# armadaproject/armada

Measured on AMD Instinct MI355X. Metric: scheduling rounds/sec (p99 round latency in p99_ms), 100k nodes x 1M jobs, higher is better.
Workload: dtype int64; 1 GPU; BASELINE configs[2]: 100000 nodes x 64 queues x 1000000 queued jobs (+560757 running), R=4, 3 priority classes, DRF weights, global burst 200000, queue burst 20000, protectedFractionOfFairShare 0.5; nodes=100000, queued_jobs=1000000, running_jobs=560757, queues=64, parallelism=1 pool on 1 gpu, seed=20260921

## Files before the change

### armada_amd/csrc/engine_hc.h

```cpp
#pragma once

#define HC_CMDS 32
#define HC_INS 16
enum { HC_Q = 1, HC_I, HC_D, HC_C, HC_E };
struct alignas(16) HcCmd { int32_t type, a; uint64_t fieldMin; int64_t ex0, ex1; int32_t cls, seq; uint64_t pad[2]; };
struct alignas(16) HcRep { int32_t seq, slot; uint64_t key; int32_t node, insDone; int64_t ex0, ex1; uint64_t cls; uint64_t pad; };
struct alignas(16) HcIns { uint64_t key; int32_t node, pad; int64_t ex0, ex1; uint64_t cls; uint64_t pad2[2]; };
struct HcBox {
  int32_t cmdPub, cmdDone, overflow, insDone;
  unsigned long long clb[128];
  int32_t scratch[64];
  int16_t freeStack[512];
  int32_t insSlot[HC_CMDS];
  HcCmd cmd[HC_CMDS]; HcRep rep[4]; HcIns ins[HC_INS];
};
static_assert(sizeof(HcCmd) == 64 && sizeof(HcRep) == 64 && sizeof(HcIns) == 64, "HC mailbox records are 64 bytes");
static_assert(sizeof(HcBox) <= sizeof(g_fl.evWin), "the HC mailbox lives in the idle key windows");
#define HCB (*(HcBox*)&g_fl.evWin[0][0])
#define HC_ROWS (L0CAP / 64)
#define HC_H_MAX 48

__device__ static inline unsigned hcMin32(unsigned v) {
  asm volatile(
      "s_nop 1\n\tv_min_u32_dpp %0, %0, %0 row_shr:1 row_mask:0xf bank_mask:0xf\n\t"
      "s_nop 1\n\tv_min_u32_dpp %0, %0, %0 row_shr:2 row_mask:0xf bank_mask:0xf\n\t"
      "s_nop 1\n\tv_min_u32_dpp %0, %0, %0 row_shr:4 row_mask:0xf bank_mask:0xf\n\t"
      "s_nop 1\n\tv_min_u32_dpp %0, %0, %0 row_shr:8 row_mask:0xf bank_mask:0xf\n\t"
      "s_nop 1\n\tv_min_u32_dpp %0, %0, %0 row_bcast:15 row_mask:0xa bank_mask:0xf\n\t"
      "s_nop 1\n\tv_min_u32_dpp %0, %0, %0 row_bcast:31 row_mask:0xc bank_mask:0xf\n\t"
      "s_nop 1"
      : "+v"(v));
  return (unsigned)__builtin_amdgcn_readlane((int)v, 63);
}
__device__ static inline unsigned long long hcMinKey(unsigned long long key, int* laneOut) {
  const unsigned hi = (unsigned)(key >> 32), lo = (unsigned)key;
  const unsigned mh = hcMin32(hi);
  const unsigned ml = hcMin32(hi == mh ? lo : 0xffffffffu);
  const unsigned long long mn = ((unsigned long long)mh << 32) | ml;
  const unsigned long long who = __ballot(key == mn);
  *laneOut = mn == ~0ull ? -1 : (int)__builtin_ctzll(who | (1ull << 63));
  return mn;
}
__device__ static inline unsigned long long hcRead64(unsigned long long v, int lane) { return slGet64(v, lane); }
__device__ static inline int hcLoadI32(const int32_t* p) { return __builtin_amdgcn_readfirstlane(__hip_atomic_load(p, __ATOMIC_RELAXED, __HIP_MEMORY_SCOPE_WORKGROUP)); }
__device__ static inline void hcStoreI32(int32_t* p, int v) { __hip_atomic_store(p, v, __ATOMIC_RELAXED, __HIP_MEMORY_SCOPE_WORKGROUP); }
struct HcNeed { unsigned long long fmin; long long ex0, ex1; int cls; };
template <int E> __device__ static inline bool hcFits(unsigned long long G, const HcNeed& q, unsigned long long key, unsigned long long cls, long long ex0, long long ex1) {
  bool ok = ((cls >> q.cls) & 1) != 0;
  ok &= (((key | G) - q.fmin) & G) == G;
  if (E > 0) ok &= q.ex0 <= ex0;
  if (E > 1) ok &= q.ex1 <= ex1;
  return ok;
}

struct HcRows { unsigned long long key[HC_ROWS], cls[HC_ROWS]; long long ex0[HC_ROWS], ex1[HC_ROWS]; };
template <int R> __device__ static inline void hcRowSet(HcRows& rows, int lane, unsigned long long key, long long ex0, long long ex1, unsigned long long cls) {
  if ((int)(threadIdx.x & 63) == lane) { rows.key[R] = key; rows.ex0[R] = ex0; rows.ex1[R] = ex1; rows.cls[R] = cls; }
}
__device__ static inline void hcRowSetAt(HcRows& rows, int slot, unsigned long long key, long long ex0, long long ex1, unsigned long long cls) {
  const int lane = slot & 63;
  switch (slot >> 6) {
#define HC_CASE(R) case R: hcRowSet<R>(rows, lane, key, ex0, ex1, cls); break;
    HC_CASE(0) HC_CASE(1) HC_CASE(2) HC_CASE(3) HC_CASE(4) HC_CASE(5) HC_CASE(6) HC_CASE(7) HC_CASE(8) HC_CASE(9) HC_CASE(10) HC_CASE(11) HC_CASE(12) HC_CASE(13) HC_CASE(14) HC_CASE(15)
#undef HC_CASE
  }
}
static_assert(HC_ROWS == 16, "hcRowSetAt enumerates the rows");

template <int E> __device__ static void coldSession(Dev& d, KREF k) {
  (void)d;
  const int lane = threadIdx.x & 63;
  const unsigned long long G = UNI64(k.guardMask);
  HcRows rows;
  int hi = __builtin_amdgcn_readfirstlane(g_fl.l0Count);
  int nfree = 0, insDone = 0, overflow = 0;
  ShapeReq sq[2];
#pragma unroll
  for (int x = 0; x < 2; x++) { const int t = lane + 64 * x; if (t < k.S) sq[x] = d.shapeTab[t]; else { sq[x].fieldMin = 0; sq[x].ex0 = sq[x].ex1 = 0; sq[x].cls = 0; sq[x].never = 1; } }
#pragma unroll
  for (int r = 0; r < HC_ROWS; r++) {
    const int s = r * 64 + lane;
    const bool in = s < hi;
    rows.key[r] = in ? g_fl.l0Key[s] : ~0ull; rows.ex0[r] = in ? g_fl.l0Ex0[s] : 0; rows.ex1[r] = in ? g_fl.l0Ex1[s] : 0; rows.cls[r] = in ? g_fl.l0Cls[s] : 0ull;
  }
  int done = 0;
  unsigned spins = 0;
  const int debugHang = d.f.debugHang;
#ifdef ASCHED_FASTPROF
  long long cBusy = 0, cT0 = 0; int cQ = 0, cI = 0;
#endif
  for (;;) {
    const HcCmd& c = HCB.cmd[done & (HC_CMDS - 1)];
    const int pubV = __hip_atomic_load(&HCB.cmdPub, __ATOMIC_RELAXED, __HIP_MEMORY_SCOPE_WORKGROUP);
    LDS_ORDER();
    const int typeV = c.type, aV = c.a, seqV = c.seq;
    HcNeed q; q.fmin = c.fieldMin; q.ex0 = c.ex0; q.ex1 = c.ex1; q.cls = c.cls;
    if (__builtin_amdgcn_readfirstlane(pubV) == done) { __builtin_amdgcn_s_sleep(1); if (waitGaveUp(spins)) return; continue; }
    spins = 0;
    if (debugHang > 0 && done == debugHang) { for (;;) { __builtin_amdgcn_s_sleep(1); if (waitGaveUp(spins)) return; } }
#ifdef ASCHED_FASTPROF
    cT0 = CLK();
#endif
    {
      const int type = __builtin_amdgcn_readfirstlane(typeV), a = __builtin_amdgcn_readfirstlane(aV);
      if (type == HC_Q) {
#ifdef ASCHED_FASTPROF
        cQ++;
#endif
        const int seq = __builtin_amdgcn_readfirstlane(seqV);
        unsigned long long best = ~0ull; int bs = -1;
        const int nrows = (hi + 63) >> 6;
#pragma unroll
        for (int rr = 0; rr < HC_ROWS; rr++) {
          if (rr < nrows) {
            const bool ok = hcFits<E>(G, q, rows.key[rr], rows.cls[rr], rows.ex0[rr], rows.ex1[rr]) & (rows.key[rr] < best);
            best = ok ? rows.key[rr] : best; bs = ok ? rr * 64 + lane : bs;
          }
        }
        int bl;
        const unsigned long long mn = hcMinKey(best, &bl);
        const int slot = bl >= 0 ? __builtin_amdgcn_readlane(bs, bl) : -1;
        HcRep& o = HCB.rep[seq & 3];
        if (lane == 0) { o.slot = slot; o.key = mn; o.insDone = overflow ? -1 : insDone; HCB.clb[a & 127] = mn; }
        LDS_ORDER();
        hcStoreI32(&o.seq, seq);
      } else if (type == HC_I) {
#ifdef ASCHED_FASTPROF
        cI++;
#endif
        const HcIns& in = HCB.ins[a & (HC_INS - 1)];
        const unsigned long long key = UNI64(in.key), cls = UNI64(in.cls); const long long ex0 = (long long)UNI64(in.ex0), ex1 = (long long)UNI64(in.ex1);
        const int node = __builtin_amdgcn_readfirstlane(in.node);
        int slot;
        if (nfree > 0) { nfree--; slot = __builtin_amdgcn_readfirstlane((int)HCB.freeStack[nfree]); }
        else if (hi < L0CAP) slot = hi++;
        else slot = -1;
        if (slot < 0) overflow = 1;
        else {
          if (lane == 0) { g_fl.l0Key[slot] = key; g_fl.l0Node[slot] = node; g_fl.l0Ex0[slot] = ex0; g_fl.l0Ex1[slot] = ex1; g_fl.l0Cls[slot] = cls; g_fl.l0Cls2[slot] = 0; HCB.insSlot[a & (HC_CMDS - 1)] = slot; }
          LANE0_PUBLISHED();
          hcRowSetAt(rows, slot, key, ex0, ex1, cls);
#pragma unroll
          for (int x = 0; x < 2; x++) {
            HcNeed nq; nq.fmin = sq[x].fieldMin; nq.ex0 = sq[x].ex0; nq.ex1 = sq[x].ex1; nq.cls = sq[x].cls;
            if (!sq[x].never && hcFits<E>(G, nq, key, cls, ex0, ex1)) (void)__hip_atomic_fetch_min(&HCB.clb[lane + 64 * x], key, __ATOMIC_RELAXED, __HIP_MEMORY_SCOPE_WORKGROUP);
          }
        }
        insDone = a + 1;
        LDS_ORDER();
        hcStoreI32(&HCB.insDone, overflow ? -1 : insDone);
      } else if (type == HC_D || type == HC_C) {
        const int slot = type == HC_D ? a : __builtin_amdgcn_readfirstlane(HCB.insSlot[a & (HC_CMDS - 1)]);
        if (slot >= 0) {
          if (lane == 0) { const int nd = g_fl.l0Node[slot]; if (nd >= 0) k.l0Slot[nd] = -1; g_fl.l0Node[slot] = -1; if (nfree < 512) HCB.freeStack[nfree] = (int16_t)slot; }
          LANE0_PUBLISHED();
          if (nfree < 512) nfree++;
          hcRowSetAt(rows, slot, ~0ull, 0, 0, 0ull);
        }
      } else if (type == HC_E) {
        int base = 0;
        const int nrows = (hi + 63) >> 6;
#pragma unroll
        for (int rr = 0; rr < HC_ROWS; rr++) {
          if (rr < nrows) {
            const int s = rr * 64 + lane;
            const int node = s < hi ? g_fl.l0Node[s] : -1;
            const bool valid = node >= 0;
            const unsigned long long b = __ballot(valid);
            const int dst = base + __popcll(b & ((1ull << lane) - 1));
            LDS_ORDER();
            if (valid) { g_fl.l0Key[dst] = rows.key[rr]; g_fl.l0Node[dst] = node; g_fl.l0Ex0[dst] = rows.ex0[rr]; g_fl.l0Ex1[dst] = rows.ex1[rr]; g_fl.l0Cls[dst] = rows.cls[rr]; g_fl.l0Cls2[dst] = 0; k.l0Slot[node] = dst; }
            LDS_ORDER();
            base += __popcll(b);
          }
        }
        if (lane == 0) g_fl.l0Count = base;
        LANE0_PUBLISHED();
#ifdef ASCHED_FASTPROF
        cBusy += CLK() - cT0;
        if (lane == 0) { g_rs.statSeg[24] += cBusy; g_rs.statSeg[25] += cQ * 1000ll; g_rs.statSeg[26] += cI * 1000ll; g_rs.statSeg[27] += (long long)hi * 1000; g_rs.statSeg[28] += 1000; }
#endif
        __builtin_amdgcn_fence(__ATOMIC_RELEASE, "agent");
        LDS_ORDER();
        hcStoreI32(&HCB.cmdDone, done + 1);
        return;
      }
      LDS_ORDER();
      done++;
    }
#ifdef ASCHED_FASTPROF
    cBusy += CLK() - cT0;
#endif
  }
}
__device__ static void coldLoop(Dev& d) {
  const FastK k = fastKRef(d);
  int gen = 0;
  unsigned spins = 0;
  for (;;) {
    for (;;) {
      int g = hcLoadI32(&g_fl.eng.hcGen);
      if (g != gen) { gen = g; break; }
      if (hcLoadI32(&g_fl.eng.bindQuit)) return;
      __builtin_amdgcn_s_sleep(2);
      if (waitGaveUp(spins)) return;
    }
    spins = 0;
    LDS_ORDER();
    if (k.E == 0) coldSession<0>(d, k); else if (k.E == 1) coldSession<1>(d, k); else coldSession<2>(d, k);
  }
}

struct HcHot { unsigned long long key, cls; long long ex0, ex1; int node, state, seq; };
enum { SC_NONE = 0, SC_SCAN = 1, SC_HEAD = 2 };
struct HcShapes { int pos[2], st[2], node[2], wIdx[2]; unsigned long long w[2], key[2], cls[2], lb[2]; long long ex0[2], ex1[2];
                  int pos2[2], node2[2]; unsigned long long key2[2], cls2[2]; long long ex02[2], ex12[2]; unsigned long long bk[2]; };
__device__ static inline void hcShapesBound(HcShapes& sc, unsigned long long on) {
#pragma unroll
  for (int x = 0; x < 2; x++) {
    const unsigned long long b = sc.st[x] == SC_HEAD ? sc.key[x] : (sc.st[x] == SC_SCAN ? sc.lb[x] : ~0ull);
    sc.bk[x] = b & on;
  }
}
__device__ static inline void hcShapesLoad(KREF k, HcShapes& sc) {
  const int lane = threadIdx.x & 63;
#pragma unroll
  for (int x = 0; x < 2; x++) {
    const int s = lane + 64 * x;
    sc.st[x] = SC_NONE; sc.pos[x] = 0; sc.node[x] = -1; sc.wIdx[x] = -1; sc.w[x] = 0; sc.key[x] = 0; sc.cls[x] = 0; sc.lb[x] = 0; sc.ex0[x] = 0; sc.ex1[x] = 0;
    sc.pos2[x] = -1; sc.node2[x] = -1; sc.key2[x] = 0; sc.cls2[x] = 0; sc.ex02[x] = 0; sc.ex12[x] = 0;
    if (s < k.S) {
      const CandRec c = g_fl.cand[s];
      if (c.node >= 0) { sc.st[x] = SC_HEAD; sc.pos[x] = c.pos; sc.node[x] = c.node; sc.key[x] = c.key; sc.cls[x] = c.cls; sc.ex0[x] = c.ex0; sc.ex1[x] = c.ex1; }
      else if (c.node == -2) { sc.st[x] = SC_SCAN; sc.pos[x] = c.pos + (c.key != 0 ? 1 : 0); sc.lb[x] = c.key; }
    }
  }
}
__device__ static inline void hcShapesStore(KREF k, const HcShapes& sc) {
  const int lane = threadIdx.x & 63;
#pragma unroll
  for (int x = 0; x < 2; x++) {
    const int s = lane + 64 * x;
    if (s < k.S) {
      CandRec c; c.pad = 0;
      if (sc.st[x] == SC_HEAD) { c.pos = sc.pos[x]; c.node = sc.node[x]; c.key = sc.key[x]; c.cls = sc.cls[x]; c.ex0 = sc.ex0[x]; c.ex1 = sc.ex1[x]; }
      else if (sc.st[x] == SC_SCAN) { c.node = -2; c.key = sc.lb[x]; c.pos = sc.lb[x] != 0 ? sc.pos[x] - 1 : sc.pos[x]; c.cls = 0; c.ex0 = c.ex1 = 0; }
      else { c.node = -1; c.pos = k.N; c.key = 0; c.cls = 0; c.ex0 = c.ex1 = 0; }
      g_fl.cand[s] = c;
    }
  }
}
__device__ static inline void hcShapesUsed(HcShapes& sc, int P) {
  const int wi = P >> 6; const unsigned long long bit = 1ull << (P & 63);
#pragma unroll
  for (int x = 0; x < 2; x++) {
    sc.w[x] = sc.wIdx[x] == wi ? sc.w[x] & ~bit : sc.w[x];
    const bool was = (sc.st[x] == SC_HEAD) & (sc.pos[x] == P);
    const bool promote = was & (sc.pos2[x] >= 0);
    const bool scan = was & !promote;
    sc.lb[x] = was ? sc.key[x] : sc.lb[x];
    sc.key[x] = promote ? sc.key2[x] : sc.key[x]; sc.cls[x] = promote ? sc.cls2[x] : sc.cls[x]; sc.node[x] = promote ? sc.node2[x] : sc.node[x];
    sc.ex0[x] = promote ? sc.ex02[x] : sc.ex0[x]; sc.ex1[x] = promote ? sc.ex12[x] : sc.ex1[x];
    sc.pos[x] = promote ? sc.pos2[x] : (scan ? P + 1 : sc.pos[x]); sc.st[x] = scan ? SC_SCAN : sc.st[x];
    sc.pos2[x] = (promote | (sc.pos2[x] == P)) ? -1 : sc.pos2[x];
  }
}
__device__ static inline void hcShapesFetch(KREF k, FastS& ES, HcShapes& sc, int target) {
  const int lane = threadIdx.x & 63;
  const int tx = target >> 6, tl = target & 63;
  for (;;) {
    unsigned long long nw[2]; bool needW[2];
#pragma unroll
    for (int x = 0; x < 2; x++) {
      const int s = lane + 64 * x, wi = sc.pos[x] >> 6;
      if (sc.st[x] == SC_SCAN && wi >= k.fitW) sc.st[x] = SC_NONE;
      needW[x] = sc.st[x] == SC_SCAN && sc.wIdx[x] != wi;
      nw[x] = 0;
      if (needW[x]) nw[x] = __hip_atomic_load(&k.fitBits[(size_t)s * k.fitW + wi], __ATOMIC_RELAXED, __HIP_MEMORY_SCOPE_AGENT);
    }
    ES.statScanSteps++;
    unsigned long long fKey[2], fCls[2]; long long fEx0[2], fEx1[2]; int fNode[2], fRem[2], hp[2]; bool needF[2];
    unsigned long long gKey[2], gCls[2]; long long gEx0[2], gEx1[2]; int gNode[2], gRem[2], hp2[2]; bool needG[2];
#pragma unroll
    for (int x = 0; x < 2; x++) {
      const int wi = sc.pos[x] >> 6;
      if (needW[x]) { sc.w[x] = nw[x]; sc.wIdx[x] = wi; }
      const unsigned long long m = sc.st[x] == SC_SCAN ? sc.w[x] & (~0ull << (sc.pos[x] & 63)) : 0ull;
      needF[x] = m != 0;
      hp[x] = wi * 64 + (int)__builtin_ctzll(m | (1ull << 63));
      if (sc.st[x] == SC_SCAN && m == 0) sc.pos[x] = (wi + 1) << 6;
      fKey[x] = 0; fCls[x] = 0; fEx0[x] = 0; fEx1[x] = 0; fNode[x] = -1; fRem[x] = 1;
      if (needF[x]) {
        const int q = hp[x];
        fRem[x] = (int)__hip_atomic_load(&k.baseRemoved[q], __ATOMIC_RELAXED, __HIP_MEMORY_SCOPE_AGENT);
        fKey[x] = k.baseKey[q]; fCls[x] = k.baseCls[q]; fNode[x] = k.baseNode[q];
        fEx0[x] = k.E > 0 ? k.baseExtra[q] : 0; fEx1[x] = k.E > 1 ? k.baseExtra[k.Npad + q] : 0;
      }
      const unsigned long long m2 = m & (m - 1);
      needG[x] = needF[x] & (m2 != 0);
      hp2[x] = wi * 64 + (int)__builtin_ctzll(m2 | (1ull << 63));
      gKey[x] = 0; gCls[x] = 0; gEx0[x] = 0; gEx1[x] = 0; gNode[x] = -1; gRem[x] = 1;
      if (needG[x]) {
        const int q = hp2[x];
        gRem[x] = (int)__hip_atomic_load(&k.baseRemoved[q], __ATOMIC_RELAXED, __HIP_MEMORY_SCOPE_AGENT);
        gKey[x] = k.baseKey[q]; gCls[x] = k.baseCls[q]; gNode[x] = k.baseNode[q];
        gEx0[x] = k.E > 0 ? k.baseExtra[q] : 0; gEx1[x] = k.E > 1 ? k.baseExtra[k.Npad + q] : 0;
      }
    }
#pragma unroll
    for (int x = 0; x < 2; x++) {
      if (needF[x]) {
        if (fRem[x]) { sc.w[x] &= ~(1ull << (hp[x] & 63)); sc.pos[x] = hp[x] + 1; }
        else {
          sc.st[x] = SC_HEAD; sc.pos[x] = hp[x]; sc.key[x] = fKey[x]; sc.cls[x] = fCls[x]; sc.node[x] = fNode[x]; sc.ex0[x] = fEx0[x]; sc.ex1[x] = fEx1[x];
          const bool sp = needG[x] & (gRem[x] == 0);
          sc.pos2[x] = sp ? hp2[x] : -1; sc.key2[x] = gKey[x]; sc.cls2[x] = gCls[x]; sc.node2[x] = gNode[x]; sc.ex02[x] = gEx0[x]; sc.ex12[x] = gEx1[x];
        }
      }
    }
    const int ts = tx ? __builtin_amdgcn_readlane(sc.st[1], tl) : __builtin_amdgcn_readlane(sc.st[0], tl);
    if (ts != SC_SCAN) return;
  }
}

struct HcJobV { unsigned long long keyDelta, fmin; long long ex0, ex1; int cls, never, rq, pub, shape; };
__device__ static inline void hcLoadEntry(int idx, HcJobV& o) {
  o.pub = __hip_atomic_load(&g_fl.eng.ringPub, __ATOMIC_RELAXED, __HIP_MEMORY_SCOPE_WORKGROUP);
  LDS_ORDER();
  o.rq = RQ(idx);
  const JobTail& t = *(const JobTail*)&RREC(idx).keyDelta;
  o.keyDelta = t.keyDelta; o.fmin = t.fieldMin; o.cls = t.cls; o.never = (int)t.never; o.ex0 = t.ex0; o.ex1 = t.ex1; o.shape = t.shape;
}
__device__ static inline void hcPostQ(int& cmdPub, const HcJobV& j, int seq) {
  HcCmd& c = HCB.cmd[cmdPub & (HC_CMDS - 1)];
  if ((threadIdx.x & 63) == 0) { c.type = HC_Q; c.a = j.shape; c.seq = seq; c.fieldMin = j.fmin; c.ex0 = j.ex0; c.ex1 = j.ex1; c.cls = j.cls; }
  LDS_ORDER();
  cmdPub++;
  hcStoreI32(&HCB.cmdPub, cmdPub);
}
__device__ static inline void hcPostA(int& cmdPub, int type, int a) {
  HcCmd& c = HCB.cmd[cmdPub & (HC_CMDS - 1)];
  if ((threadIdx.x & 63) == 0) { c.type = type; c.a = a; }
  LDS_ORDER();
  cmdPub++;
  hcStoreI32(&HCB.cmdPub, cmdPub);
}

__device__ static inline int hcHotBind(HcHot& h, int hLane, const HcJobV& j, unsigned long long G, unsigned long long MFM, long long ME0, long long ME1) {
  const unsigned long long nk = h.key - j.keyDelta; const long long n0 = h.ex0 - j.ex0, n1 = h.ex1 - j.ex1;
  const bool alive = ((((nk | G) - MFM) & G) == G) & (ME0 <= n0) & (ME1 <= n1);
  const bool me = (int)(threadIdx.x & 63) == hLane;
  h.key = me ? (alive ? nk : ~0ull) : h.key; h.ex0 = me ? n0 : h.ex0; h.ex1 = me ? n1 : h.ex1; h.state = me ? (alive ? 1 : 0) : h.state; h.cls = (me & !alive) ? 0ull : h.cls;
  return __ballot(me & !alive) ? 1 : 0;
}
#define HC_ERR_SHORT 610

struct HcOut { int engSeq, statScanSteps, statL0Max, hcShort; long long segT, eseg[8]; };
template <int E> __device__ static __attribute__((noinline)) HcOut engineStreamHcT(Dev& d, const FastK k, const int engSeq0, const int statScan0, const int statL0Max0, const long long segT0) {
  FastS ES; ES.engSeq = engSeq0; ES.statScanSteps = statScan0; ES.statL0Max = statL0Max0; ES.segT = segT0; ES.laneL = 0; ES.laneX = 0;
#ifdef ASCHED_FASTPROF
  for (int x = 0; x < 8; x++) ES.eseg[x] = 0;
#endif
  const int lane = threadIdx.x & 63;
  const unsigned long long G = UNI64(k.guardMask), MFM = UNI64(k.minFieldMin);
  const long long ME0 = (long long)UNI64(k.minEx0), ME1 = (long long)UNI64(k.minEx1);
  if (lane == 0) { HCB.cmdPub = 0; HCB.cmdDone = 0; HCB.overflow = 0; HCB.insDone = 0; for (int x = 0; x < 4; x++) HCB.rep[x].seq = -1; }
  HCB.clb[lane] = 0; HCB.clb[lane + 64] = 0;
  LDS_ORDER();
  hcStoreI32(&g_fl.eng.hcGen, __builtin_amdgcn_readfirstlane(g_fl.eng.hcGen) + 1);
  int cmdPub = 0, insSeq = 0, rrNext = 0, qSeq = 0, inFlight = 0;
  HcHot h; h.key = ~0ull; h.cls = 0; h.ex0 = h.ex1 = 0; h.node = -1; h.state = 0; h.seq = 0;
  const unsigned long long shortOn = d.f.hcShort ? ~0ull : 0ull;
  HcShapes sc; hcShapesLoad(k, sc); hcShapesBound(sc, shortOn);
  int nShort = 0;
  int total = __builtin_amdgcn_readfirstlane(g_fl.l0Count);
  int i = 0, fail = 0;
  HcJobV cur; bool haveCur = false;
#ifdef ASCHED_FASTPROF
  int pSrc[4] = {0, 0, 0, 0}, pFetch = 0, pDry = 0, pAsk = 0;
#endif
#ifdef ASCHED_HC_CHECK
  int chkNode = -1, chkQ = 0, chkScan = 0;
#endif
  for (;;) {
    if (!haveCur) {
#ifdef ASCHED_FASTPROF
      pDry++;
#endif
      for (;;) {
        hcLoadEntry(i, cur);
        if (__builtin_amdgcn_readfirstlane(cur.pub) > i) break;
        if (hcLoadI32(&g_fl.eng.ringEnd) | hcLoadI32(&g_fl.eng.abandon)) { hcLoadEntry(i, cur); break; }
        __builtin_amdgcn_s_sleep(1);
      }
      if (__builtin_amdgcn_readfirstlane(cur.pub) <= i) break;
      haveCur = true;
    }
    ESEG(0);
    const int flags = __builtin_amdgcn_readfirstlane((cur.rq & RQ_EV) | (cur.never << 16));
    if (flags) {
      if (flags >> 16) { fail = 1; break; }
      i++; haveCur = false;
      hcStoreI32(&g_fl.eng.ringAck, i);
      continue;
    }
    if ((++ES.engSeq & 255) == 0 && cancelRequested(d)) { if (lane == 0) g_fl.eng.cancel = 1; LANE0_PUBLISHED(); fail = 1; break; }
    HcJobV nxt; hcLoadEntry(i + 1, nxt);
    const int rIns = __hip_atomic_load(&HCB.insDone, __ATOMIC_RELAXED, __HIP_MEMORY_SCOPE_WORKGROUP);
    LDS_ORDER();
    const unsigned long long rLb = HCB.clb[cur.shape & 127];
    HcNeed q; q.fmin = cur.fmin; q.ex0 = cur.ex0; q.ex1 = cur.ex1; q.cls = cur.cls;
    const bool fitH = hcFits<E>(G, q, h.key, h.cls, h.ex0, h.ex1);
    int hLane;
    unsigned long long hk = hcMinKey(fitH ? h.key : ~0ull, &hLane);
    const int shape = __builtin_amdgcn_readfirstlane(cur.shape), sl = shape & 63;
    const bool hiSet = cur.shape >= 64;
    ESEG(1);
    int insDone = __builtin_amdgcn_readfirstlane(rIns);
    if (insDone < 0) { fail = 2; break; }
    if (inFlight > 0) {
      const bool rel = (h.state == 2) & (h.seq < insDone);
      const unsigned long long rb = __ballot(rel);
      h.state = rel ? 0 : h.state; h.cls = rel ? 0ull : h.cls; h.key = rel ? ~0ull : h.key;
      inFlight -= __popcll(rb);
      const bool drop = hLane >= 0 && ((rb >> hLane) & 1);
      hLane = drop ? -1 : hLane; hk = drop ? ~0ull : hk;
    }
    {
      const unsigned long long bkS = hcRead64(hiSet ? sc.bk[1] : sc.bk[0], sl);
      const int stH = __builtin_amdgcn_readlane(h.state, hLane & 63);
#ifdef ASCHED_HC_CHECK
      chkNode = -1; chkQ = qSeq; chkScan = ES.statScanSteps;
      if (!(rLb < hk) & (hk < bkS) & (stH == 1)) chkNode = __builtin_amdgcn_readlane(h.node, hLane & 63);
#else
      if (!(rLb < hk) & (hk < bkS) & (stH == 1)) {
        RREC(i).node0 = __builtin_amdgcn_readlane(h.node, hLane & 63);
        LDS_ORDER();
        i++;
        hcStoreI32(&g_fl.eng.ringAck, i);
        total -= hcHotBind(h, hLane, cur, G, MFM, ME0, ME1);
        nShort++;
        cur = nxt; haveCur = __builtin_amdgcn_readfirstlane(nxt.pub) > i;
        ESEG(6);
        continue;
      }
#endif
    }
    int cst = __builtin_amdgcn_readlane(hiSet ? sc.st[1] : sc.st[0], sl);
    unsigned long long cKey = hcRead64(hiSet ? sc.key[1] : sc.key[0], sl);
    const unsigned long long cLb = hcRead64(hiSet ? sc.lb[1] : sc.lb[0], sl);
    const unsigned long long ckLb = UNI64(rLb);
    const unsigned long long known = cst == SC_HEAD && cKey < hk ? cKey : hk;
    unsigned long long ck = ~0ull; int cSlot = -1;
    if (ckLb < known) {
#ifdef ASCHED_FASTPROF
      pAsk++;
#endif
      hcPostQ(cmdPub, cur, qSeq);
      HcRep& rp = HCB.rep[qSeq & 3];
      for (;;) { if ((int)(hcLoadI32(&rp.seq) == qSeq) | hcLoadI32(&g_fl.eng.abandon)) break; __builtin_amdgcn_s_sleep(1); }
      LDS_ORDER();
      qSeq++;
      cSlot = __builtin_amdgcn_readfirstlane(rp.slot); ck = UNI64(rp.key);
      insDone = __builtin_amdgcn_readfirstlane(rp.insDone) | -hcLoadI32(&g_fl.eng.abandon);
      if (insDone < 0) { fail = 2; break; }
      const bool rel = (h.state == 2) & (h.seq < insDone);
      const unsigned long long rb = __ballot(rel);
      h.state = rel ? 0 : h.state; h.cls = rel ? 0ull : h.cls; h.key = rel ? ~0ull : h.key;
      inFlight -= __popcll(rb);
      const bool drop = hLane >= 0 && ((rb >> hLane) & 1);
      hLane = drop ? -1 : hLane; hk = drop ? ~0ull : hk;
    }
    ESEG(2);
    const unsigned long long lk = hk < ck ? hk : ck;
    if (cst == SC_SCAN && !(lk < cLb)) {
#ifdef ASCHED_FASTPROF
      pFetch++;
#endif
      hcShapesFetch(k, ES, sc, shape);
      hcShapesBound(sc, shortOn);
      cst = __builtin_amdgcn_readlane(hiSet ? sc.st[1] : sc.st[0], sl);
      cKey = hcRead64(hiSet ? sc.key[1] : sc.key[0], sl);
    }
    const unsigned long long lk2 = hk < ck ? hk : ck;
    const unsigned long long bk = cst == SC_HEAD ? cKey : (cst == SC_SCAN ? cLb : ~0ull);
    const bool dirtyWins = lk2 < bk;
    if (!dirtyWins & (cst != SC_HEAD)) { fail = 1; break; }
    const int src = dirtyWins ? (hk < ck ? 0 : 1) : 2;
    const int nH = __builtin_amdgcn_readlane(h.node, hLane & 63), nB = __builtin_amdgcn_readlane(hiSet ? sc.node[1] : sc.node[0], sl);
    int n = dirtyWins ? nH : nB;
    if (src == 1) n = __builtin_amdgcn_readfirstlane(g_fl.l0Node[cSlot]);
#ifdef ASCHED_HC_CHECK
    if (chkNode >= 0) {
      if ((src != 0) | (n != chkNode) | (qSeq != chkQ) | (ES.statScanSteps != chkScan)) { if (lane == 0 && RS.error == 0) { RS.error = ASCHED_ERR_INTERNAL; RS.errorDetail = HC_ERR_SHORT; } LANE0_PUBLISHED(); fail = 1; break; }
      nShort++;
    }
#endif
#ifdef ASCHED_FASTPROF
    pSrc[src & 3]++;
#endif
    ESEG(3);
    RREC(i).node0 = n;
    LDS_ORDER();
    i++;
    hcStoreI32(&g_fl.eng.ringAck, i);
    if (src == 1) hcPostA(cmdPub, HC_D, cSlot);
    if (inFlight > 0 && src == 0 && __builtin_amdgcn_readlane(h.state, hLane) == 2) { hcPostA(cmdPub, HC_C, __builtin_amdgcn_readlane(h.seq, hLane)); inFlight--; }
    const bool haveNext = __builtin_amdgcn_readfirstlane(nxt.pub) > i;
    ESEG(4);
    if (src == 0) {
      total -= hcHotBind(h, hLane, cur, G, MFM, ME0, ME1);
    } else {
      unsigned long long okey, ocls; long long oex0, oex1;
      if (src == 1) { okey = ck; ocls = UNI64(g_fl.l0Cls[cSlot]); oex0 = (long long)UNI64(g_fl.l0Ex0[cSlot]); oex1 = (long long)UNI64(g_fl.l0Ex1[cSlot]); }
      else {
        okey = cKey;
        ocls = hcRead64(hiSet ? sc.cls[1] : sc.cls[0], sl);
        oex0 = (long long)hcRead64((unsigned long long)(hiSet ? sc.ex0[1] : sc.ex0[0]), sl);
        oex1 = (long long)hcRead64((unsigned long long)(hiSet ? sc.ex1[1] : sc.ex1[0]), sl);
        const int usedPos = __builtin_amdgcn_readlane(hiSet ? sc.pos[1] : sc.pos[0], sl);
        baseMarkRemoved(k, ES, usedPos);
        hcShapesUsed(sc, usedPos);
        hcShapesBound(sc, shortOn);
      }
      const unsigned long long nk = okey - UNI64(cur.keyDelta); const long long n0 = oex0 - (long long)UNI64(cur.ex0), n1 = oex1 - (long long)UNI64(cur.ex1);
      const bool alive = ((((nk | G) - MFM) & G) == G) && ME0 <= n0 && ME1 <= n1;
      if (alive) {
        const unsigned long long occ = __ballot(h.state != 0);
        if (occ == ~0ull) { fail = 2; break; }
        const int fl = (int)__builtin_ctzll(~occ);
        const bool me = lane == fl;
        h.key = me ? nk : h.key; h.cls = me ? ocls : h.cls; h.ex0 = me ? n0 : h.ex0; h.ex1 = me ? n1 : h.ex1; h.node = me ? n : h.node; h.state = me ? 1 : h.state;
        if (src != 1) { total++; if (total > ES.statL0Max) ES.statL0Max = total; }
        const unsigned long long normal = __ballot(h.state == 1);
        if (__popcll(normal) > HC_H_MAX) {
          while (insSeq - insDone >= HC_INS / 2) {
            __builtin_amdgcn_s_sleep(1);
            insDone = hcLoadI32(&HCB.insDone) | -hcLoadI32(&g_fl.eng.abandon);
            if (insDone < 0) break;
          }
          if (insDone < 0) { fail = 2; break; }
          const unsigned long long cand = normal & ~(1ull << fl);
          const unsigned long long hiPart = cand & (~0ull << rrNext);
          const int v = hiPart ? (int)__builtin_ctzll(hiPart) : (int)__builtin_ctzll(cand);
          rrNext = (v + 1) & 63;
          HcIns& in = HCB.ins[insSeq & (HC_INS - 1)];
          if (lane == v) { in.key = h.key; in.node = h.node; in.ex0 = h.ex0; in.ex1 = h.ex1; in.cls = h.cls; }
          h.state = lane == v ? 2 : h.state; h.seq = lane == v ? insSeq : h.seq;
          LDS_ORDER();
          hcPostA(cmdPub, HC_I, insSeq);
          insSeq++; inFlight++;
        }
      } else if (src == 1) total--;
    }
    cur = nxt; haveCur = haveNext;
    ESEG(5);
  }
  bool gaveUp = waitAbandoned();
  if (gaveUp) fail = 1;
#ifdef ASCHED_FASTPROF
  if (lane == 0) { g_rs.statSeg[29] += pSrc[0] * 1000ll; g_rs.statSeg[30] += pSrc[1] * 1000ll; g_rs.statSeg[31] += pSrc[2] * 1000ll; g_rs.statSeg[33] += pFetch * 1000ll; g_rs.statSeg[35] += pDry * 1000ll; g_rs.statSeg[36] += pAsk * 1000ll; g_rs.statSeg[32] += nShort * 1000ll; }
#endif
  hcShapesStore(k, sc);
  if (!gaveUp) {
    hcPostA(cmdPub, HC_E, 0);
    for (;;) { if (hcLoadI32(&HCB.cmdDone) == cmdPub) break; __builtin_amdgcn_s_sleep(1); if (waitAbandoned()) { gaveUp = true; break; } }
  }
  LDS_ORDER();
  if (!gaveUp) {
    int cnt = __builtin_amdgcn_readfirstlane(g_fl.l0Count);
    const bool mine = h.state == 1;
    const unsigned long long b = __ballot(mine);
    const int dst = cnt + __popcll(b & ((1ull << lane) - 1));
    const int add = __popcll(b);
    if (cnt + add > L0CAP) { if (fail != 1) fail = 2; else fail = 3; }
    else {
      if (mine) { g_fl.l0Key[dst] = h.key; g_fl.l0Node[dst] = h.node; g_fl.l0Ex0[dst] = h.ex0; g_fl.l0Ex1[dst] = h.ex1; g_fl.l0Cls[dst] = h.cls; g_fl.l0Cls2[dst] = 0; k.l0Slot[h.node] = dst; }
      if (lane == 0) g_fl.l0Count = cnt + add;
      LANE0_PUBLISHED();
    }
  }
  if (fail == 3) fail = 2;
  if (fail) { LDS_ORDER(); hcStoreI32(&g_fl.eng.ringFail, fail); }
  HcOut o; o.engSeq = ES.engSeq; o.statScanSteps = ES.statScanSteps; o.statL0Max = ES.statL0Max; o.hcShort = nShort; o.segT = ES.segT;
  for (int x = 0; x < 8; x++) o.eseg[x] = 0;
#ifdef ASCHED_FASTPROF
  for (int x = 0; x < 8; x++) o.eseg[x] = ES.eseg[x];
#endif
  return o;
}
__device__ static inline void engineStreamHc(Dev& d, KREF k, FastS& ES) {
  HcOut o;
  if (k.E == 0) o = engineStreamHcT<0>(d, k, ES.engSeq, ES.statScanSteps, ES.statL0Max, ES.segT); else if (k.E == 1) o = engineStreamHcT<1>(d, k, ES.engSeq, ES.statScanSteps, ES.statL0Max, ES.segT); else o = engineStreamHcT<2>(d, k, ES.engSeq, ES.statScanSteps, ES.statL0Max, ES.segT);
  ES.engSeq = o.engSeq; ES.statScanSteps = o.statScanSteps; ES.statL0Max = o.statL0Max;
  if ((threadIdx.x & 63) == 0) g_rs.statHcShort += o.hcShort;
  LANE0_PUBLISHED();
#ifdef ASCHED_FASTPROF
  ES.segT = o.segT; for (int x = 0; x < 8; x++) ES.eseg[x] += o.eseg[x];
#endif
}
```

Before: 4.591 rounds/s.

## Track per-lane rank masks for hot-cache pick instead of DPP min reduction

Each lane of the hot cache now keeps a 64-bit mask of which lanes hold a smaller key. The fitting minimum is then found with ballots and a single first-lane test instead of a two-pass DPP 64-bit min reduction. The masks are updated on every insert, rebind and release, which adds ballot work to those paths. A debug check compares the result against the old min path. Tie handling differs when keys are equal, which the check would flag.

```diff
diff --git a/armada_amd/csrc/engine_hc.h b/armada_amd/csrc/engine_hc.h
--- a/armada_amd/csrc/engine_hc.h
+++ b/armada_amd/csrc/engine_hc.h
@@ -1,4 +1,5 @@
 #pragma once
+#include "hc_order.h"
 
 #define HC_CMDS 32
 #define HC_INS 16
@@ -52,6 +53,13 @@
   if (E > 1) ok &= q.ex1 <= ex1;
   return ok;
 }
+template <int E> __device__ static inline unsigned long long hcFitsMask(unsigned long long G, const HcNeed& q, unsigned long long key, unsigned long long cls, long long ex0, long long ex1) {
+  unsigned long long m = __builtin_amdgcn_ballot_w64(((cls >> q.cls) & 1) != 0);
+  m &= __builtin_amdgcn_ballot_w64((((key | G) - q.fmin) & G) == G);
+  if (E > 0) m &= __builtin_amdgcn_ballot_w64(q.ex0 <= ex0);
+  if (E > 1) m &= __builtin_amdgcn_ballot_w64(q.ex1 <= ex1);
+  return m;
+}
 
 struct HcRows { unsigned long long key[HC_ROWS], cls[HC_ROWS]; long long ex0[HC_ROWS], ex1[HC_ROWS]; };
 template <int R> __device__ static inline void hcRowSet(HcRows& rows, int lane, unsigned long long key, long long ex0, long long ex1, unsigned long long cls) {
@@ -211,7 +219,18 @@
   }
 }
 
-struct HcHot { unsigned long long key, cls; long long ex0, ex1; int node, state, seq; };
+struct HcHot { unsigned long long key, cls, below; long long ex0, ex1; int node, state, seq; };
+__device__ static inline unsigned long long hcOrderPick(const HcHot& h, unsigned long long fitMask, int* laneOut) {
+  const unsigned long long who = __builtin_amdgcn_ballot_w64(hcOrderFirst(true, h.below, fitMask)) & fitMask;
+  const int l = (int)__builtin_ctzll(who | (1ull << 63));
+  const unsigned long long kl = hcRead64(h.key, l);
+  *laneOut = who ? l : -1;
+  return who ? kl : ~0ull;
+}
+__device__ static inline void hcOrderSet(HcHot& h, int L, unsigned long long nk) {
+  const unsigned long long lt = __builtin_amdgcn_ballot_w64(h.key < nk);
+  h.below = hcOrderUpdate(h.below, h.key, (int)(threadIdx.x & 63), __builtin_amdgcn_readfirstlane(L), nk, lt);
+}
 enum { SC_NONE = 0, SC_SCAN = 1, SC_HEAD = 2 };
 struct HcShapes { int pos[2], st[2], node[2], wIdx[2]; unsigned long long w[2], key[2], cls[2], lb[2]; long long ex0[2], ex1[2];
                   int pos2[2], node2[2]; unsigned long long key2[2], cls2[2]; long long ex02[2], ex12[2]; unsigned long long bk[2]; };
@@ -351,9 +370,12 @@
   const bool alive = ((((nk | G) - MFM) & G) == G) & (ME0 <= n0) & (ME1 <= n1);
   const bool me = (int)(threadIdx.x & 63) == hLane;
   h.key = me ? (alive ? nk : ~0ull) : h.key; h.ex0 = me ? n0 : h.ex0; h.ex1 = me ? n1 : h.ex1; h.state = me ? (alive ? 1 : 0) : h.state; h.cls = (me & !alive) ? 0ull : h.cls;
-  return __ballot(me & !alive) ? 1 : 0;
+  const unsigned long long nkL = hcRead64(h.key, hLane);
+  hcOrderSet(h, hLane, nkL);
+  return nkL == ~0ull ? 1 : 0;
 }
 #define HC_ERR_SHORT 610
+#define HC_ERR_ORDER 611
 
 struct HcOut { int engSeq, statScanSteps, statL0Max, hcShort; long long segT, eseg[8]; };
 template <int E> __device__ static __attribute__((noinline)) HcOut engineStreamHcT(Dev& d, const FastK k, const int engSeq0, const int statScan0, const int statL0Max0, const long long segT0) {
@@ -369,7 +391,7 @@
   LDS_ORDER();
   hcStoreI32(&g_fl.eng.hcGen, __builtin_amdgcn_readfirstlane(g_fl.eng.hcGen) + 1);
   int cmdPub = 0, insSeq = 0, rrNext = 0, qSeq = 0, inFlight = 0;
-  HcHot h; h.key = ~0ull; h.cls = 0; h.ex0 = h.ex1 = 0; h.node = -1; h.state = 0; h.seq = 0;
+  HcHot h; h.key = ~0ull; h.cls = 0; h.below = 0; h.ex0 = h.ex1 = 0; h.node = -1; h.state = 0; h.seq = 0;
   const unsigned long long shortOn = d.f.hcShort ? ~0ull : 0ull;
   HcShapes sc; hcShapesLoad(k, sc); hcShapesBound(sc, shortOn);
   int nShort = 0;
@@ -410,9 +432,20 @@
     LDS_ORDER();
     const unsigned long long rLb = HCB.clb[cur.shape & 127];
     HcNeed q; q.fmin = cur.fmin; q.ex0 = cur.ex0; q.ex1 = cur.ex1; q.cls = cur.cls;
+    int hLane;
+#ifdef ASCHED_HC_DPPMIN
     const bool fitH = hcFits<E>(G, q, h.key, h.cls, h.ex0, h.ex1);
-    int hLane;
     unsigned long long hk = hcMinKey(fitH ? h.key : ~0ull, &hLane);
+#else
+    unsigned long long hk = hcOrderPick(h, hcFitsMask<E>(G, q, h.key, h.cls, h.ex0, h.ex1), &hLane);
+#endif
+#ifdef ASCHED_HC_CHECK
+    {
+      int mLane; const unsigned long long mk = hcMinKey(hcFits<E>(G, q, h.key, h.cls, h.ex0, h.ex1) ? h.key : ~0ull, &mLane);
+      int oLane; const unsigned long long ok = hcOrderPick(h, hcFitsMask<E>(G, q, h.key, h.cls, h.ex0, h.ex1), &oLane);
+      if ((mLane != oLane) | (mk != ok)) { if (lane == 0 && RS.error == 0) { RS.error = ASCHED_ERR_INTERNAL; RS.errorDetail = HC_ERR_ORDER; } LANE0_PUBLISHED(); fail = 1; break; }
+    }
+#endif
     const int shape = __builtin_amdgcn_readfirstlane(cur.shape), sl = shape & 63;
     const bool hiSet = cur.shape >= 64;
     ESEG(1);
@@ -422,6 +455,7 @@
       const bool rel = (h.state == 2) & (h.seq < insDone);
       const unsigned long long rb = __ballot(rel);
       h.state = rel ? 0 : h.state; h.cls = rel ? 0ull : h.cls; h.key = rel ? ~0ull : h.key;
+      h.below = hcOrderRelease(h.below, rb);
       inFlight -= __popcll(rb);
       const bool drop = hLane >= 0 && ((rb >> hLane) & 1);
       hLane = drop ? -1 : hLane; hk = drop ? ~0ull : hk;
@@ -467,6 +501,7 @@
       const bool rel = (h.state == 2) & (h.seq < insDone);
       const unsigned long long rb = __ballot(rel);
       h.state = rel ? 0 : h.state; h.cls = rel ? 0ull : h.cls; h.key = rel ? ~0ull : h.key;
+      h.below = hcOrderRelease(h.below, rb);
       inFlight -= __popcll(rb);
       const bool drop = hLane >= 0 && ((rb >> hLane) & 1);
       hLane = drop ? -1 : hLane; hk = drop ? ~0ull : hk;
@@ -530,6 +565,7 @@
         if (occ == ~0ull) { fail = 2; break; }
         const int fl = (int)__builtin_ctzll(~occ);
         const bool me = lane == fl;
+        hcOrderSet(h, fl, nk);
         h.key = me ? nk : h.key; h.cls = me ? ocls : h.cls; h.ex0 = me ? n0 : h.ex0; h.ex1 = me ? n1 : h.ex1; h.node = me ? n : h.node; h.state = me ? 1 : h.state;
         if (src != 1) { total++; if (total > ES.statL0Max) ES.statL0Max = total; }
         const unsigned long long normal = __ballot(h.state == 1);
diff --git a/armada_amd/csrc/hc_order.h b/armada_amd/csrc/hc_order.h
--- /dev/null
+++ b/armada_amd/csrc/hc_order.h
@@ -0,0 +1,19 @@
+#pragma once
+#include <stdint.h>
+
+#if defined(__HIPCC__) || defined(__CUDACC__)
+#define HC_ORDER_FN __host__ __device__ static inline
+#else
+#define HC_ORDER_FN static inline
+#endif
+
+HC_ORDER_FN bool hcOrderFirst(bool fit, uint64_t below, uint64_t fitMask) { return fit & ((below & fitMask) == 0); }
+
+HC_ORDER_FN uint64_t hcOrderUpdate(uint64_t below, uint64_t key, int lane, int L, uint64_t nk, uint64_t lt) {
+  const uint64_t bitL = (uint64_t)1 << L;
+  const uint64_t sel = (uint64_t)0 - (uint64_t)(nk < key);
+  const uint64_t others = below ^ ((below ^ sel) & bitL);
+  return lane == L ? (lt & ~bitL) : others;
+}
+
+HC_ORDER_FN uint64_t hcOrderRelease(uint64_t below, uint64_t rb) { return below & ~rb; }
```

Result: faster. 4.672 rounds/s, median of 6 (+1.8%).
